# SutirthaChakraborty/RTFS-Net

Measured on AMD Instinct MI355X. Metric: mixtures/sec forward (2 s@16 kHz, 2-spk) RTFS-Net-4, higher is better.
Workload: dtype f32 (f16x3 split-precision MFMA products, f32 accumulate; every tensor in HBM is f32)

## Files before the change

rtfs-net_amd/csrc/api.hip:

```cpp
#include "api_common.h"
#include <atomic>
#include <vector>

namespace {

struct Cursor {
    const float* p;
    size_t off = 0;
    explicit Cursor(const float* base) : p(base) {}
    const float* take(size_t n) {
        const float* r = p ? p + off : nullptr;
        off += (n + 63) / 64 * 64;
        return r;
    }
};

struct Fork {
    hipStream_t st = nullptr;
    RtfsSide side{};
    bool open = false;
    int begin(hipStream_t owner, int slot) {
        st = owner;
        CHECK(rtfs_side_stream(owner, slot, &side));
        if (hipEventRecord(side.fork, st) != hipSuccess || hipStreamWaitEvent(side.stream, side.fork, 0) != hipSuccess) return RTFS_ERR_LAUNCH;
// ... 148 lines not shown
    explicit DecPack(Cursor& c) {
        wt = c.take(CA * 32);
        w16 = c.take(CA * 32);
        w16p = c.take(8192);
    }
};

inline bool gemm_f32() {
    static const bool v = [] {
        const char* e = getenv("RTFS_GEMM_F32");
        return e && e[0] == '1';
    }();
    return v;
}

DpArgs dp_args(const DpPack& p, const float* x, float* out, int R, int Ls, size_t bstride, size_t rstride, size_t cstride) {
    DpArgs a;
    a.x = x;
    a.out = out;
    a.R = R;
    a.Ls = Ls;
    a.bstride = bstride;
    a.rstride = rstride;
    a.cstride = cstride;
    a.ln_gamma = p.ln_g;
    a.ln_beta = p.ln_b;
    a.W0 = p.W0;
    a.Wl = p.Wl;
    a.wc = p.wc;
    a.bias = p.bias;
    a.Wt = p.Wt;
    a.bt = p.bt;
    a.whh = p.whh;
    return a;
}

Dp16Args dp16_args(const DpPack& p, const float* x, float* out, int nseq, int R, int Ls, size_t bstride, size_t rstride, size_t cstride) {
    Dp16Args a;
    a.x = x;
    a.out = out;
    a.nseq = nseq;
    a.R = R;
    a.Ls = Ls;
    a.bstride = bstride;
    a.rstride = rstride;
    a.cstride = cstride;
    a.ln_gamma = p.ln_g;
    a.ln_beta = p.ln_b;
    a.w16_l0 = reinterpret_cast<const half8*>(p.w16_l0);
    a.w16_l = reinterpret_cast<const half8*>(p.w16_l);
    a.w16_ct = reinterpret_cast<const half8*>(p.w16_ct);
    a.wf_l0 = reinterpret_cast<const half8*>(p.wf_l0);
    a.wf_l = reinterpret_cast<const half8*>(p.wf_l);
    a.wf_ct = reinterpret_cast<const half8*>(p.wf_ct);
    a.wc16 = p.wc16;
    a.bias16 = p.bias16;
    a.bt = p.bt;
    return a;
}

int dualpath(const DpPack& p, const float* x, float* out, int B, int T, int F, int dim, float* tA, float* tB, hipStream_t st) {
    const size_t plane = (size_t)T * F;
    if (dim == 4) {
        RTFS_RETURN_IF(F < 8 || F > 250, RTFS_ERR_SHAPE);
        if (!gemm_f32() && !p.whh) return launch_dualpath16(dp16_args(p, x, out, B * T, T, F, CH * plane, F, plane), st);
        return launch_dualpath(dp_args(p, x, out, T, F, CH * plane, F, plane), B * T, st);
    }
    RTFS_RETURN_IF(T < 8 || T > (p.whh ? 250 : 512), RTFS_ERR_SHAPE);
    CHECK(launch_transpose(x, tA, B * CH, T, F, st));
    if (T > 256 && !p.whh) {
        const int nb = (int)std::min<size_t>((size_t)B, (((size_t)1 << 32) - 1) / (CH * plane * sizeof(float)));
        for (int b0 = 0; b0 < B; b0 += nb) {
            const int n = std::min(nb, B - b0);
            CHECK(launch_dualpath16(dp16_args(p, tA + (size_t)b0 * CH * plane, tB + (size_t)b0 * CH * plane, n * F, F, T, CH * plane, T, plane), st));
        }
    } else if ((!gemm_f32() || T > 250) && !p.whh) {
        CHECK(launch_dualpath16(dp16_args(p, tA, tB, B * F, F, T, CH * plane, T, plane), st));
    } else {
        CHECK(launch_dualpath(dp_args(p, tA, tB, F, T, CH * plane, T, plane), B * F, st));
    }
    return launch_transpose(tB, out, B * CH, F, T, st);
}

int attention(const AttnPack& p, const float* x, float* out, int B, int T, float* q, float* k, float* v, float* o, hipStream_t st, bool cl = false) {
    RowCanArgs a;
    a.x = x;
    a.cl = cl;
    a.wt = p.qkv_wt;
    a.bias = p.qkv_b;
    a.slope = p.qkv_slope;
    a.gamma = p.qkv_gamma;
    a.beta = p.qkv_beta;
    a.ngroups = 12;
    for (int g = 0; g <= 12; ++g) a.group_start[g] = g <= 8 ? 4 * g : 32 + 16 * (g - 8);
    for (int g = 0; g < 12; ++g)
        for (int o_ = a.group_start[g]; o_ < a.group_start[g + 1]; ++o_) a.group_of[o_] = (unsigned char)g;
    a.T = T;
    a.q = q;
    a.k = k;
    a.v = v;
    CHECK(launch_row_can_qkv(a, B, st));
    AttnArgs c;
    c.q = q;
    c.k = k;
    c.v = v;
    c.out = o;
    c.T = T;
    c.scale = 1.0f / 16.0f;
    CHECK(launch_attn_core(c, B, st));
    RowCanArgs r;
    r.x = o;
    r.wt = p.proj_wt;
    r.bias = p.proj_b;
    r.slope = p.proj_slope;
    r.gamma = p.proj_gamma;
    r.beta = p.proj_beta;
    r.ngroups = 1;
    r.group_start[0] = 0;
    r.group_start[1] = 64;
    r.T = T;
    r.res = x;
    r.cl = cl;
    r.out = out;
    return launch_row_can_proj(r, B, st);
}

struct BlockWs {
    float *residual, *x_enc, *c0, *xf0, *expanded;
    float *c1, *p0, *g, *gF, *tA, *tB, *gT, *gA, *q, *k, *v, *o;
    float *E0, *G0, *E1, *G1, *L1, *xf1, *E2, *G2;
    double* stats;
    int Bfull = 0;
    int cs = 0;
    static constexpr int NSTAT = 11;
    enum { S_C0, S_C1, S_E0, S_G0, S_E1, S_G1, S_L1, S_E2, S_G2, S_L0, S_L2 };
    BlockWs(Arena& a, int B, int T, int F, int cs_ = 0) {
        const size_t Pg = (size_t)(T / 2) * (F / 2);
        cs = cs_ ? cs_ : T * F;
        const size_t P = (size_t)cs;
        Bfull = B;
        residual = a.take<float>(B * CA * P);
        x_enc = a.take<float>(B * CH * P);
        c0 = a.take<float>(B * CH * P);
        xf0 = a.take<float>(B * CH * P);
        expanded = a.take<float>(B * CH * P);
        float** gs[] = {&c1, &p0, &g, &gF, &tA, &tB, &gT, &gA, &v, &o, &E0, &G0, &E1, &G1, &L1, &xf1, &E2, &G2};
        for (float** s : gs) *s = a.take<float>(B * CH * Pg);
        q = a.take<float>(B * CH * Pg / 4);
        k = a.take<float>(B * CH * Pg / 4);
        stats = a.take<double>((size_t)NSTAT * B * 2);
    }
    double* st(int slot, int ) const { return stats ? stats + (size_t)slot * Bfull * 2 : nullptr; }
};

int block_head(const BlockPack& p, const float* x, const float* x_res, int B, int T, int F, BlockWs& w, hipStream_t st, const CafArgs* caf, unsigned* ctr = nullptr) {
    const int P = T * F;
    {
        PwArgs a;
        a.x = x;
        a.x2 = x_res;
        a.res_out = w.residual;
        a.wt = p.proj_wt;
        a.w16 = p.proj_w16;
        a.bias = p.proj_b;
        a.out = w.x_enc;
        a.gw = p.gw;
        a.gb = p.gb;
        a.slope = p.gslope;
        a.P = P;
        a.cs = w.cs;
        a.tile_ctr = ctr;
        if (caf && !gemm_f32()) {
            a.caf_r = caf->r_out; a.caf_att = caf->att_out;
            a.caf_w_key = caf->w_key; a.caf_bn_key = caf->bn_key; a.caf_w_val = caf->w_val; a.caf_bn_val = caf->bn_val;
            a.caf_T = caf->T; a.caf_F = caf->F; a.caf_Tv = caf->Tv;
        }
        if (gemm_f32()) return launch_pw_gateway_proj(a, B, st);
        const int rc = launch_pws_head4(a, B, st);
        if (rc == RTFS_ERR_ARG) CHECK(launch_pws_gateway_proj(a, B, st));
        else CHECK(rc);
    }
    return RTFS_OK;
}

int block_body(const BlockPack& p, int B, int T, int F, const BlockWs& w, hipStream_t st, bool zero_stats = true) {
    const int Tp = T / 2, Fp = F / 2;
    const int P = T * F, Pg = Tp * Fp;
    const double icF = 1.0 / ((double)CH * P), icG = 1.0 / ((double)CH * Pg);
    typedef BlockWs W;
    constexpr int TH_A = 24, TH_B = 24, TH_C = 12, TH_G = 64, TH_S = 64;
    if (zero_stats && hipMemsetAsync(w.stats, 0, sizeof(double) * W::NSTAT * w.Bfull * 2, st) != hipSuccess) return RTFS_ERR_LAUNCH;
    {
        DwArgs a;
        a.x = w.x_enc;
        a.w[0] = p.ds0_w;
        a.bias[0] = p.ds0_b;
        a.out[0] = w.c0;
        a.stats_out[0] = w.st(W::S_C0, B);
        a.C = CH; a.H = T; a.W = F; a.TH = TH_A; a.cs = w.cs;
        CHECK(launch_dw_s1(a, 1, false, 0, B, st));
    }
    DwArgs s14;
    s14.x = w.c0;
    s14.in_stats = w.st(W::S_C0, B); s14.in_inv_count = icF; s14.in_gamma = p.ds0_g; s14.in_beta = p.ds0_be;
    s14.C = CH; s14.H = T; s14.W = F; s14.TH = 64; s14.Hg = Tp; s14.Wg = Fp; s14.cs = w.cs;
    s14.w[0] = p.fus0.loc_w;
    s14.stats_out[0] = w.st(W::S_L0, B);
    s14.rev = 1;
    DwArgs s3;
    s3.x = w.c0;
    s3.in_stats = w.st(W::S_C0, B); s3.in_inv_count = icF; s3.in_gamma = p.ds0_g; s3.in_beta = p.ds0_be;
    s3.w[0] = p.ds1_w;
    s3.bias[0] = p.ds1_b;
    s3.out[0] = w.c1;
    s3.out[1] = w.p0;
    s3.stats_out[0] = w.st(W::S_C1, B);
    s3.C = CH; s3.H = T; s3.W = F; s3.Hg = Tp; s3.Wg = Fp; s3.TH = TH_C; s3.cs = w.cs;
    s3.rev = 1;
    {
        const int rc = launch_dw_s2_stats(s3, s14, B, st);
        if (rc != RTFS_OK) return rc == RTFS_ERR_ARG ? RTFS_ERR_SHAPE : rc;
    }
    CHECK(launch_g_form(w.p0, w.c1, w.st(W::S_C1, B), icG, p.ds1_g, p.ds1_be, w.g, B, CH, Pg, st));
    const size_t per = (size_t)CH * Pg;
    const int nb = (int)std::min<size_t>((size_t)B, (((size_t)1 << 32) - 1) / (per * sizeof(float)));
    const bool cl = !p.dpF.whh && !p.dpT.whh && !gemm_f32() && !dualpath_gen2() && Fp >= 8 && Fp <= 64 && Tp >= 8 && Tp <= 512 &&
                    nb >= 1 && (nb >= B || Tp > 256);
    if (cl) {
        for (int b0 = 0; b0 < B; b0 += nb) {
            const int n = std::min(nb, B - b0);
// ... 264 lines not shown
        case RTFS_PACK_ATTENTION: return pack_size<AttnPack>();
        case RTFS_PACK_TFAR: return pack_size<TfarPack>();
        case RTFS_PACK_CAF: return pack_size<CafPack>();
        case RTFS_PACK_S3: return pack_size<S3Pack>();
        case RTFS_PACK_DECODER: return pack_size<DecPack>();
    }
    return 0;
}

size_t rtfs_stft_encoder_workspace_bytes(int B, int L) { return (size_t)B * 2 * rtfs_num_frames(L) * NF * sizeof(float) + 256; }

int rtfs_stft_encoder_f32(const float* wav, const float* pack, float* a0, double* stats, int B, int L, void* ws, size_t ws_bytes, void* stream) {
    RTFS_RETURN_IF(!wav || !pack || !a0 || B < 1 || L <= 128, RTFS_ERR_ARG);
    const int T = rtfs_num_frames(L);
    Arena ar(ws, ws_bytes);
    float* spec = ar.take<float>((size_t)B * 2 * T * NF);
    RTFS_RETURN_IF(!ws || !ar.ok(), RTFS_ERR_WORKSPACE);
    Cursor c(pack);
    EncPack p(c);
    if (stats && hipMemsetAsync(stats, 0, sizeof(double) * 2 * B, S(stream)) != hipSuccess) return RTFS_ERR_LAUNCH;
    CHECK(launch_stft(wav, spec, B, L, T, S(stream)));
    return launch_enc_conv(spec, p.w, a0, stats, B, CA, T, NF, (size_t)T * NF, (size_t)CA * T * NF, S(stream));
}

size_t rtfs_audio_bottleneck_workspace_bytes(int B) { return sizeof(double) * 2 * B + 256; }

int rtfs_audio_bottleneck_f32(const float* x, const double* stats, const float* pack, float* out, int B, int T, int F, void* ws, size_t ws_bytes, void* stream) {
    RTFS_RETURN_IF(!x || !pack || !out || B < 1 || T < 1 || F < 1, RTFS_ERR_ARG);
    Cursor c(pack);
    BnPack p(c);
    if (!stats) {
        Arena ar(ws, ws_bytes);
        double* s = ar.take<double>(2 * B);
        RTFS_RETURN_IF(!ws || !ar.ok(), RTFS_ERR_WORKSPACE);
        if (hipMemsetAsync(s, 0, sizeof(double) * 2 * B, S(stream)) != hipSuccess) return RTFS_ERR_LAUNCH;
        CHECK(launch_stats(x, s, B, (size_t)CA * T * F, S(stream)));
        stats = s;
    }
    return audio_bn(p, x, stats, out, B, T * F, S(stream));
}

size_t rtfs_block_workspace_bytes(int B, int T, int F) {
    Arena ar(nullptr, 0);
    BlockWs w(ar, B, T, F);
    return ar.off + 256;
}

int rtfs_block_f32(const float* x, const float* x_res, const float* pack, float* out, int B, int T, int F, void* ws, size_t ws_bytes, void* stream, int rnn_kind) {
    RTFS_RETURN_IF(!x || !pack || !out, RTFS_ERR_ARG);
    RTFS_RETURN_IF(!shape_ok_block(B, T, F, rnn_kind), RTFS_ERR_SHAPE);
    Arena ar(ws, ws_bytes);
    BlockWs w(ar, B, T, F);
    RTFS_RETURN_IF(!ws || !ar.ok(), RTFS_ERR_WORKSPACE);
    RTFS_RETURN_IF(rnn_kind != 0 && rnn_kind != 1, RTFS_ERR_ARG);
    Cursor c(pack);
    BlockPack p = BlockPack::make(c, rnn_kind);
    return block_forward(p, x, x_res, out, B, T, F, w, S(stream));
}

size_t rtfs_dualpath_workspace_bytes(int B, int T, int F) { return 2 * ((size_t)B * CH * T * F * sizeof(float) + 256); }

int rtfs_dualpath_lstm_f32(const float* x, const float* pack, float* out, int B, int T, int F, int dim, void* ws, size_t ws_bytes, void* stream) {
    RTFS_RETURN_IF(!x || !pack || !out || B < 1 || (dim != 3 && dim != 4), RTFS_ERR_ARG);
    Arena ar(ws, ws_bytes);
    float* tA = ar.take<float>((size_t)B * CH * T * F);
    float* tB = ar.take<float>((size_t)B * CH * T * F);
    RTFS_RETURN_IF(dim == 3 && (!ws || !ar.ok()), RTFS_ERR_WORKSPACE);
    Cursor c(pack);
    DpPack p(c, 1);
    return dualpath(p, x, out, B, T, F, dim, tA, tB, S(stream));
}

int rtfs_dualpath_sru_f32(const float* x, const float* pack, float* out, int B, int T, int F, int dim, void* ws, size_t ws_bytes, void* stream) {
    RTFS_RETURN_IF(!x || !pack || !out || B < 1 || (dim != 3 && dim != 4), RTFS_ERR_ARG);
    Arena ar(ws, ws_bytes);
    float* tA = ar.take<float>((size_t)B * CH * T * F);
    float* tB = ar.take<float>((size_t)B * CH * T * F);
    RTFS_RETURN_IF(dim == 3 && (!ws || !ar.ok()), RTFS_ERR_WORKSPACE);
    Cursor c(pack);
    DpPack p(c);
    return dualpath(p, x, out, B, T, F, dim, tA, tB, S(stream));
}

size_t rtfs_tf_attention_workspace_bytes(int B, int T) { return (size_t)B * T * (4 * 256 + 4 * 256 + 4 * 1024 + 64 * FQ) * sizeof(float) + 4 * 256; }

int rtfs_tf_attention_f32(const float* x, const float* pack, float* out, int B, int T, void* ws, size_t ws_bytes, void* stream) {
    RTFS_RETURN_IF(!x || !pack || !out || B < 1, RTFS_ERR_ARG);
    RTFS_RETURN_IF(T < 1 || T > 512, RTFS_ERR_SHAPE);
    Arena ar(ws, ws_bytes);
    float* q = ar.take<float>((size_t)B * 4 * T * 256);
    float* k = ar.take<float>((size_t)B * 4 * T * 256);
    float* v = ar.take<float>((size_t)B * 4 * T * 1024);
    float* o = ar.take<float>((size_t)B * 64 * T * FQ);
    RTFS_RETURN_IF(!ws || !ar.ok(), RTFS_ERR_WORKSPACE);
    Cursor c(pack);
    AttnPack p(c);
    return attention(p, x, out, B, T, q, k, v, o, S(stream));
}

size_t rtfs_tfar_workspace_bytes(int B, int H, int W, int Hg, int Wg) {
    return 3 * ((size_t)B * CH * (size_t)(H * W > Hg * Wg ? Hg * Wg : H * W) * sizeof(float) + 256) + 3 * 2 * B * sizeof(double) + 256;
}

int rtfs_tfar_f32(const float* local, const float* global, const float* pack, float* out, int B, int H, int W, int Hg, int Wg, void* ws, size_t ws_bytes, void* stream) {
    RTFS_RETURN_IF(!local || !global || !pack || !out || B < 1, RTFS_ERR_ARG);
    const bool up = (size_t)H * W > (size_t)Hg * Wg;
    RTFS_RETURN_IF(!up && (H != Hg || W != Wg), RTFS_ERR_SHAPE);
    Arena ar(ws, ws_bytes);
    const size_t ng = (size_t)B * CH * Hg * Wg;
    float* E = ar.take<float>(ng);
    float* G = ar.take<float>(ng);
    float* Lc = ar.take<float>(ng);
    double* st = ar.take<double>(3 * 2 * B);
    RTFS_RETURN_IF(!ws || !ar.ok(), RTFS_ERR_WORKSPACE);
    Cursor c(pack);
    TfarPack p(c);
    hipStream_t s = S(stream);
    if (hipMemsetAsync(st, 0, sizeof(double) * 6 * B, s) != hipSuccess) return RTFS_ERR_LAUNCH;
    double *stE = st, *stG = st + 2 * B, *stL = st + 4 * B;
    const double icG = 1.0 / ((double)CH * Hg * Wg), icL = 1.0 / ((double)CH * H * W);
    {
        DwArgs a;
        a.x = global;
        a.w[0] = p.emb_w; a.w[1] = p.gate_w;
        a.out[0] = E; a.out[1] = G;
        a.stats_out[0] = stE; a.stats_out[1] = stG;
        a.C = CH; a.H = Hg; a.W = Wg; a.TH = 64;
        CHECK(launch_dw_s1(a, 2, false, 0, B, s));
    }
    if (up) {
        DwArgs a;
        a.x = local;
        a.w[0] = p.loc_w;
        a.C = CH; a.H = H; a.W = W; a.TH = 64; a.Hg = Hg; a.Wg = Wg;
        a.stats_out[0] = stL;
        CHECK(launch_dw_s1(a, 1, false, 1, B, s));
        a.stats_out[0] = nullptr;
        a.loc_stats = stL; a.loc_inv_count = icL; a.loc_gamma = p.loc_g; a.loc_beta = p.loc_b;
        a.gate = G; a.gate_stats = stG; a.gate_gamma = p.gate_g; a.gate_beta = p.gate_b;
        a.emb = E; a.emb_stats = stE; a.emb_gamma = p.emb_g; a.emb_beta = p.emb_b;
        a.g_inv_count = icG;
        a.out[0] = out;
        return launch_dw_s1(a, 1, false, 2, B, s);
    }
    {
        DwArgs a;
        a.x = local;
        a.w[0] = p.loc_w;
        a.out[0] = Lc;
        a.stats_out[0] = stL;
        a.C = CH; a.H = H; a.W = W; a.TH = 64;
        CHECK(launch_dw_s1(a, 1, false, 0, B, s));
    }
    GCombineArgs a;
    a.l = Lc; a.gate = G; a.emb = E;
    a.l_stats = stL; a.gate_stats = stG; a.emb_stats = stE;
    a.l_gamma = p.loc_g; a.l_beta = p.loc_b; a.gate_gamma = p.gate_g; a.gate_beta = p.gate_b; a.emb_gamma = p.emb_g; a.emb_beta = p.emb_b;
    a.inv_count = icG;
    a.out = out;
    a.C = CH; a.HW = H * W;
    return launch_g_combine(a, B, s);
}

size_t rtfs_caf_workspace_bytes(int B, int Tv) { return 2 * ((size_t)B * CA * Tv * sizeof(float) + 256); }

int rtfs_caf_f32(const float* audio, const float* video, const float* pack, float* out, int B, int T, int F, int Tv, void* ws, size_t ws_bytes, void* stream) {
    RTFS_RETURN_IF(!audio || !video || !pack || !out || B < 1 || T < 1 || F < 1 || Tv < 1, RTFS_ERR_ARG);
    Arena ar(ws, ws_bytes);
    float* r = ar.take<float>((size_t)B * CA * Tv);
    float* att = ar.take<float>((size_t)B * CA * Tv);
    RTFS_RETURN_IF(!ws || !ar.ok(), RTFS_ERR_WORKSPACE);
    Cursor c(pack);
    CafPack p(c);
    CafArgs a = caf_args(p, audio, video, out, r, att, T, F, Tv);
    CHECK(launch_caf_video(a, B, S(stream)));
// ... 410 lines not shown
```

rtfs-net_amd/csrc/k_attn.hip:

```cpp
#include "common.h"
#include "kernels.h"
#include "pipe_helpers.h"

#define AF 64

#define RCAN_ROWS 8
#define RCAN_LD 72
template <int NOUT, bool CL = false>
__global__ __launch_bounds__(256, 2) void row_can_kernel(RowCanArgs a) {
    constexpr int MT = NOUT / 32, MTW = (MT + 1) / 2;
    constexpr int NR = NOUT / 4;
    constexpr float WSC = 256.f, WINV = 1.f / 256.f;
    __shared__ float Ys[NOUT][RCAN_LD];
    __shared__ float bias_s[NOUT], slope_s[NOUT];
    __shared__ float red[8];
    constexpr bool XCL = CL && NOUT == 96, RCL = CL && NOUT == 64;
    __shared__ __attribute__((aligned(16))) float Rs[RCL ? AF : 1][RCL ? 68 : 4];
    const int T = a.T, b = blockIdx.y;
    const int tid = threadIdx.x, lane = tid & 63, r = lane & 31, h = lane >> 5;
    const int wave = __builtin_amdgcn_readfirstlane(tid >> 6);
    const int nt = wave & 1, mp = wave >> 1;
    for (int o = tid; o < NOUT; o += 256) {
        bias_s[o] = a.bias[o] * WSC;
        slope_s[o] = a.slope[NOUT == 96 ? a.group_of[o] : 0];
    }
    half8 wh[MTW][4], wl[MTW][4];
#pragma unroll
    for (int m = 0; m < MTW; ++m) {
        const int mt = min(mp + 2 * m, MT - 1);
#pragma unroll
        for (int ks = 0; ks < 4; ++ks)
#pragma unroll
            for (int j = 0; j < 8; ++j) {
                const float w = a.wt[(ks * 16 + 8 * h + j) * NOUT + mt * 32 + r] * WSC;
                const _Float16 hi = (_Float16)w;
                wh[m][ks][j] = hi;
                wl[m][ks][j] = (_Float16)(w - (float)hi);
            }
    }
    auto ln_row = [&](int i) -> int {
        if (NOUT == 64) return wave * 16 + i;
        return i < 4 ? 4 * wave + i : i < 8 ? 16 + 4 * wave + (i - 4) : 32 + 16 * wave + (i - 8);
    };
    __shared__ float gam_s[NOUT][AF], bet_s[NOUT][AF];
    for (int i = tid; i < NOUT * AF; i += 256) {
        gam_s[0][i] = a.gamma[i];
        bet_s[0][i] = a.beta[i];
    }
    const int t0 = blockIdx.x * a.rpw;
    const int nrows = min(a.rpw, T - t0);
    const float* __restrict__ X = XCL ? a.x + ((size_t)b * T * AF + nt * 32 + r) * 64 + 8 * h : a.x + (size_t)b * 64 * T * AF + nt * 32 + r;
    const float* __restrict__ RES = NOUT == 64 ? (RCL ? a.res + (size_t)b * T * AF * 64 + 4 * tid : a.res + ((size_t)b * 64 + wave * 16) * T * AF + lane)
                                               : nullptr;
    float v[4][8];
    float rs[NOUT == 64 ? 16 : 1];
    auto load_x = [&](int t) {
        if constexpr (XCL) {
#pragma unroll
            for (int ks = 0; ks < 4; ++ks) {
                *reinterpret_cast<f32x4*>(&v[ks][0]) = *reinterpret_cast<const f32x4*>(X + (size_t)t * AF * 64 + ks * 16);
                *reinterpret_cast<f32x4*>(&v[ks][4]) = *reinterpret_cast<const f32x4*>(X + (size_t)t * AF * 64 + ks * 16 + 4);
            }
        } else {
#pragma unroll
            for (int ks = 0; ks < 4; ++ks)
#pragma unroll
                for (int j = 0; j < 8; ++j) v[ks][j] = X[((size_t)(ks * 16 + 8 * h + j) * T + t) * AF];
        }
    };
    load_x(t0);
    __syncthreads();
    for (int rr = 0; rr < nrows; ++rr) {
        const int t = t0 + rr;
        half8 bh[4], bl[4];
#pragma unroll
        for (int ks = 0; ks < 4; ++ks) {
            unsigned hi[4], lo[4];
#pragma unroll
            for (int jp = 0; jp < 4; ++jp) split2(v[ks][2 * jp], v[ks][2 * jp + 1], hi[jp], lo[jp]);
            bh[ks] = __builtin_bit_cast(half8, *reinterpret_cast<f32x4*>(hi));
            bl[ks] = __builtin_bit_cast(half8, *reinterpret_cast<f32x4*>(lo));
        }
        if constexpr (RCL) {
#pragma unroll
            for (int k = 0; k < 4; ++k) *reinterpret_cast<f32x4*>(&rs[4 * k]) = *reinterpret_cast<const f32x4*>(RES + (size_t)t * AF * 64 + 1024 * k);
        } else if (NOUT == 64) {
#pragma unroll
            for (int i = 0; i < 16; ++i) rs[i] = RES[((size_t)i * T + t) * AF];
        }
        load_x(min(t + 1, T - 1));
#pragma unroll
        for (int m = 0; m < MTW; ++m) {
            const int mt = mp + 2 * m;
            if (mt < MT) {
                f32x16 acc;
#pragma unroll
                for (int q = 0; q < 16; ++q) acc[q] = bias_s[mt * 32 + (q & 3) + 8 * (q >> 2) + 4 * h];
#pragma unroll
                for (int ks = 0; ks < 4; ++ks) {
                    acc = __builtin_amdgcn_mfma_f32_32x32x16_f16(wh[m][ks], bh[ks], acc, 0, 0, 0);
                    acc = __builtin_amdgcn_mfma_f32_32x32x16_f16(wh[m][ks], bl[ks], acc, 0, 0, 0);
                    acc = __builtin_amdgcn_mfma_f32_32x32x16_f16(wl[m][ks], bh[ks], acc, 0, 0, 0);
                }
#pragma unroll
                for (int q = 0; q < 16; ++q) {
                    const int o = mt * 32 + (q & 3) + 8 * (q >> 2) + 4 * h;
                    Ys[o][nt * 32 + r] = preluf_(acc[q] * WINV, slope_s[o]);
                }
            }
        }
        if constexpr (RCL) {
#pragma unroll
            for (int k = 0; k < 4; ++k) *reinterpret_cast<f32x4*>(&Rs[tid / 16 + 16 * k][4 * (tid % 16)]) = *reinterpret_cast<const f32x4*>(&rs[4 * k]);
        }
        __syncthreads();
        float y[NR];
#pragma unroll
        for (int i = 0; i < NR; ++i) y[i] = Ys[ln_row(i)][lane];
        if (NOUT == 96) {
#pragma unroll
            for (int g = 0; g < 3; ++g) {
                const int i0 = g == 0 ? 0 : g == 1 ? 4 : 8, gs = g == 2 ? 16 : 4;
                float s = 0.f;
#pragma unroll
                for (int i = 0; i < gs; ++i) s += y[i0 + i];
                const float mean = wave_sum(s) / (float)(gs * AF);
                float vv = 0.f;
#pragma unroll
                for (int i = 0; i < gs; ++i) {
                    y[i0 + i] -= mean;
                    vv = fmaf(y[i0 + i], y[i0 + i], vv);
                }
                const float rstd = 1.0f / sqrtf(wave_sum(vv) / (float)(gs * AF) + RTFS_EPS);
                float* __restrict__ dst = (g == 0 ? a.q : g == 1 ? a.k : a.v) + (((size_t)b * 4 + wave) * T + t) * (gs * AF) + lane;
#pragma unroll
                for (int i = 0; i < gs; ++i) dst[i * AF] = fmaf(y[i0 + i] * rstd, gam_s[ln_row(i0 + i)][lane], bet_s[ln_row(i0 + i)][lane]);
            }
        } else {
            float s = 0.f;
#pragma unroll
            for (int i = 0; i < 16; ++i) s += y[i];
            s = wave_sum(s);
            if (lane == 0) red[wave] = s;
            __syncthreads();
            const float mean = (red[0] + red[1] + red[2] + red[3]) / (float)(64 * AF);
            float vv = 0.f;
#pragma unroll
            for (int i = 0; i < 16; ++i) {
                y[i] -= mean;
                vv = fmaf(y[i], y[i], vv);
            }
            vv = wave_sum(vv);
            if (lane == 0) red[4 + wave] = vv;
            __syncthreads();
            const float rstd = 1.0f / sqrtf((red[4] + red[5] + red[6] + red[7]) / (float)(64 * AF) + RTFS_EPS);
            float* __restrict__ O = a.out + ((size_t)b * 64 + wave * 16) * T * AF + lane;
            if constexpr (RCL) {
#pragma unroll
                for (int k = 0; k < 4; ++k) *reinterpret_cast<f32x4*>(&rs[4 * k]) = *reinterpret_cast<const f32x4*>(&Rs[lane][wave * 16 + 4 * k]);
            }
#pragma unroll
            for (int i = 0; i < 16; ++i) O[((size_t)i * T + t) * AF] = fmaf(y[i] * rstd, gam_s[ln_row(i)][lane], bet_s[ln_row(i)][lane]) + rs[i];
        }
        __syncthreads();
    }
}

#define ATT_PSC 4096.f
__device__ __forceinline__ void split8(const float (&v)[8], float sc, half8& hi, half8& lo) {
    unsigned h[4], l[4];
#pragma unroll
    for (int jp = 0; jp < 4; ++jp) split2(v[2 * jp] * sc, v[2 * jp + 1] * sc, h[jp], l[jp]);
    hi = __builtin_bit_cast(half8, *reinterpret_cast<f32x4*>(h));
    lo = __builtin_bit_cast(half8, *reinterpret_cast<f32x4*>(l));
}
__global__ __launch_bounds__(256) void attn_core_kernel(AttnArgs a) {
    extern __shared__ __attribute__((aligned(16))) float S[];
    const int T = a.T;
    const int NKT = (T + 31) >> 5;
    const int NK = NKT * 32;
    const int ldp = NK + 4;
    const int tid = threadIdx.x, lane = tid & 63, r = lane & 31, h = lane >> 5;
    const int wave = __builtin_amdgcn_readfirstlane(tid >> 6);
    const int nqt = (T + 31) >> 5;
    const int slot = blockIdx.x >> 3;
    const int pair = (slot / nqt) * 8 + (blockIdx.x & 7);
    if (pair >= a.npairs) return;
    const int q0 = (slot % nqt) * 32, hd = pair & 3, b = pair >> 2;
    const float* __restrict__ Q = a.q + ((size_t)b * 4 + hd) * T * 256;
    const float* __restrict__ K = a.k + ((size_t)b * 4 + hd) * T * 256;
    const float* __restrict__ V = a.v + ((size_t)b * 4 + hd) * T * 1024;

    for (int kg = 0; kg < NKT; kg += 8) {
        f32x16 acc[2];
#pragma unroll
        for (int j = 0; j < 2; ++j)
#pragma unroll
            for (int q = 0; q < 16; ++q) acc[j][q] = 0.f;
        const float* __restrict__ qp = Q + (size_t)min(q0 + r, T - 1) * 256 + 8 * h;
        const float* __restrict__ kp0 = K + (size_t)min((kg + wave) * 32 + r, T - 1) * 256 + 8 * h;
        const float* __restrict__ kp1 = K + (size_t)min((kg + wave + 4) * 32 + r, T - 1) * 256 + 8 * h;
        const bool two = kg + wave + 4 < NKT;
#pragma unroll 4
        for (int ks = 0; ks < 16; ++ks) {
            float qv[8], k0[8], k1[8];
            *reinterpret_cast<f32x4*>(qv) = *reinterpret_cast<const f32x4*>(qp + ks * 16);
            *reinterpret_cast<f32x4*>(qv + 4) = *reinterpret_cast<const f32x4*>(qp + ks * 16 + 4);
            *reinterpret_cast<f32x4*>(k0) = *reinterpret_cast<const f32x4*>(kp0 + ks * 16);
            *reinterpret_cast<f32x4*>(k0 + 4) = *reinterpret_cast<const f32x4*>(kp0 + ks * 16 + 4);
            *reinterpret_cast<f32x4*>(k1) = *reinterpret_cast<const f32x4*>(kp1 + ks * 16);
            *reinterpret_cast<f32x4*>(k1 + 4) = *reinterpret_cast<const f32x4*>(kp1 + ks * 16 + 4);
            half8 ah, al, bh, bl;
            split8(qv, 1.f, ah, al);
            split8(k0, 1.f, bh, bl);
            acc[0] = __builtin_amdgcn_mfma_f32_32x32x16_f16(ah, bh, acc[0], 0, 0, 0);
            acc[0] = __builtin_amdgcn_mfma_f32_32x32x16_f16(ah, bl, acc[0], 0, 0, 0);
            acc[0] = __builtin_amdgcn_mfma_f32_32x32x16_f16(al, bh, acc[0], 0, 0, 0);
            if (two) {
                split8(k1, 1.f, bh, bl);
                acc[1] = __builtin_amdgcn_mfma_f32_32x32x16_f16(ah, bh, acc[1], 0, 0, 0);
                acc[1] = __builtin_amdgcn_mfma_f32_32x32x16_f16(ah, bl, acc[1], 0, 0, 0);
                acc[1] = __builtin_amdgcn_mfma_f32_32x32x16_f16(al, bh, acc[1], 0, 0, 0);
            }
        }
#pragma unroll
        for (int j = 0; j < 2; ++j) {
            const int kt = kg + wave + 4 * j;
            if (kt < NKT) {
#pragma unroll
                for (int q = 0; q < 16; ++q) S[((q & 3) + 8 * (q >> 2) + 4 * h) * ldp + kt * 32 + r] = acc[j][q] * a.scale;
            }
        }
    }
    __syncthreads();
    for (int rr = 0; rr < 8; ++rr) {
        float* row = S + (wave * 8 + rr) * ldp;
        float m = -3.0e38f;
        for (int j = lane; j < T; j += 64) m = fmaxf(m, row[j]);
        m = wave_max(m);
        float s = 0.f;
        for (int j = lane; j < NK; j += 64) {
            const float e = j < T ? expf(row[j] - m) : 0.f;
            row[j] = e;
            s += e;
        }
        const float inv = 1.0f / wave_sum(s);
        for (int j = lane; j < NK; j += 64) row[j] *= inv;
    }
    __syncthreads();
    for (int grp = 0; grp < 2; ++grp) {
        f32x16 o[4];
#pragma unroll
        for (int n = 0; n < 4; ++n)
#pragma unroll
            for (int q = 0; q < 16; ++q) o[n][q] = 0.f;
        const int col0 = (wave * 8 + grp * 4) * 32 + 4 * r;
        const float* __restrict__ vp = V + col0;
        f32x4 vv[2][8];
        auto load_v = [&](int ks, f32x4 (&dst)[8]) {
#pragma unroll
            for (int j = 0; j < 8; ++j) dst[j] = *reinterpret_cast<const f32x4*>(vp + (size_t)min(ks * 16 + 8 * h + j, T - 1) * 1024);
        };
        auto step = [&](int ks, const f32x4 (&src)[8]) {
            float pv[8];
            *reinterpret_cast<f32x4*>(pv) = *reinterpret_cast<const f32x4*>(S + r * ldp + ks * 16 + 8 * h);
            *reinterpret_cast<f32x4*>(pv + 4) = *reinterpret_cast<const f32x4*>(S + r * ldp + ks * 16 + 8 * h + 4);
            half8 ph, pl;
            split8(pv, ATT_PSC, ph, pl);
#pragma unroll
            for (int n = 0; n < 4; ++n) {
                float t8[8];
#pragma unroll
                for (int j = 0; j < 8; ++j) t8[j] = src[j][n];
                half8 vh, vl;
                split8(t8, 1.f, vh, vl);
                o[n] = __builtin_amdgcn_mfma_f32_32x32x16_f16(ph, vh, o[n], 0, 0, 0);
                o[n] = __builtin_amdgcn_mfma_f32_32x32x16_f16(ph, vl, o[n], 0, 0, 0);
                o[n] = __builtin_amdgcn_mfma_f32_32x32x16_f16(pl, vh, o[n], 0, 0, 0);
            }
        };
        const int nks = NK / 16;
        load_v(0, vv[0]);
        for (int ks = 0; ks < nks; ks += 2) {
            load_v(ks + 1, vv[1]);
            step(ks, vv[0]);
            load_v(min(ks + 2, nks - 1), vv[0]);
            step(ks + 1, vv[1]);
        }
        {
            const int c = col0 >> 6, f = col0 & 63;
#pragma unroll
            for (int q = 0; q < 16; ++q) {
                const int qq = q0 + (q & 3) + 8 * (q >> 2) + 4 * h;
                if (qq < T)
                    *reinterpret_cast<f32x4*>(a.out + (((size_t)b * 64 + hd * 16 + c) * T + qq) * AF + f) =
                        f32x4{o[0][q], o[1][q], o[2][q], o[3][q]} * (1.f / ATT_PSC);
            }
        }
    }
}

size_t attn_core_lds_bytes(int T) {
    const int NK = ((T + 31) >> 5) * 32;
    return (size_t)32 * (NK + 4) * sizeof(float);
}

static int rcan_rows(int T, int B) {
    if ((long)T * B >= 3500) return RCAN_ROWS;
    const int r = (int)((long)T * B / 512);
    return r < 1 ? 1 : (r > RCAN_ROWS ? RCAN_ROWS : r);
}
int launch_row_can_qkv(const RowCanArgs& a_, int B, hipStream_t st) {
    RowCanArgs a = a_;
    a.rpw = rcan_rows(a.T, B);
    if (a.ngroups != 12 || a.group_start[8] != 32 || a.group_start[12] != 96) return RTFS_ERR_SHAPE;
    if (a.cl)
        hipLaunchKernelGGL((row_can_kernel<96, true>), dim3(cdiv(a.T, a.rpw), B), dim3(256), 0, st, a);
    else
        hipLaunchKernelGGL((row_can_kernel<96, false>), dim3(cdiv(a.T, a.rpw), B), dim3(256), 0, st, a);
    return rtfs_launch_status();
}
int launch_row_can_proj(const RowCanArgs& a_, int B, hipStream_t st) {
    RowCanArgs a = a_;
    a.rpw = rcan_rows(a.T, B);
    if (a.ngroups != 1) return RTFS_ERR_SHAPE;
    if (a.cl)
        hipLaunchKernelGGL((row_can_kernel<64, true>), dim3(cdiv(a.T, a.rpw), B), dim3(256), 0, st, a);
    else
        hipLaunchKernelGGL((row_can_kernel<64, false>), dim3(cdiv(a.T, a.rpw), B), dim3(256), 0, st, a);
    return rtfs_launch_status();
}
int launch_attn_core(const AttnArgs& a, int B, hipStream_t st) {
    if (a.T < 1 || a.T > 512) return RTFS_ERR_SHAPE;
    const size_t lds = attn_core_lds_bytes(a.T);
    if (rtfs_set_max_lds((const void*)attn_core_kernel, lds) != RTFS_OK) return RTFS_ERR_LAUNCH;
    AttnArgs a2 = a;
    a2.npairs = B * 4;
    hipLaunchKernelGGL(attn_core_kernel, dim3(cdiv(a2.npairs, 8) * 8 * cdiv(a.T, 32)), dim3(256), lds, st, a2);
    return rtfs_launch_status();
}
```

Measured before the change: 3308.

## Store attention Q/K/V pre-split as fp16 hi/lo pairs and restructure attention core

The QKV projection kernel now writes Q and K as interleaved fp16 hi/lo halves and V as row-paired fp16 hi/lo words, so the attention core no longer re-splits f32 values on every MFMA step. The attention core loads half8 operands directly, software-pipelines QK^T over K chunks, prefetches V three stages ahead, and stores softmax probabilities in LDS as fp16 hi/lo. The output projection now reads a transposed attention output layout. The aim is to cut the VALU split work and memory traffic in attention, at the cost of more complex layouts, higher register pressure with two blocks per CU, and odd-T handling in the V packing.

```diff
diff --git a/rtfs-net_amd/csrc/api.hip b/rtfs-net_amd/csrc/api.hip
--- a/rtfs-net_amd/csrc/api.hip
+++ b/rtfs-net_amd/csrc/api.hip
@@ -254,6 +254,7 @@
     return launch_transpose(tB, out, B * CH, F, T, st);
 }
 
+static size_t attn_v_rows(int T) { return ((size_t)T + 1) & ~(size_t)1; }
 int attention(const AttnPack& p, const float* x, float* out, int B, int T, float* q, float* k, float* v, float* o, hipStream_t st, bool cl = false) {
     RowCanArgs a;
     a.x = x;
@@ -316,8 +317,9 @@
         c0 = a.take<float>(B * CH * P);
         xf0 = a.take<float>(B * CH * P);
         expanded = a.take<float>(B * CH * P);
-        float** gs[] = {&c1, &p0, &g, &gF, &tA, &tB, &gT, &gA, &v, &o, &E0, &G0, &E1, &G1, &L1, &xf1, &E2, &G2};
+        float** gs[] = {&c1, &p0, &g, &gF, &tA, &tB, &gT, &gA, &o, &E0, &G0, &E1, &G1, &L1, &xf1, &E2, &G2};
         for (float** s : gs) *s = a.take<float>(B * CH * Pg);
+        v = a.take<float>(B * CH * attn_v_rows(T / 2) * (F / 2));
         q = a.take<float>(B * CH * Pg / 4);
         k = a.take<float>(B * CH * Pg / 4);
         stats = a.take<double>((size_t)NSTAT * B * 2);
@@ -748,7 +750,9 @@
     return dualpath(p, x, out, B, T, F, dim, tA, tB, S(stream));
 }
 
-size_t rtfs_tf_attention_workspace_bytes(int B, int T) { return (size_t)B * T * (4 * 256 + 4 * 256 + 4 * 1024 + 64 * FQ) * sizeof(float) + 4 * 256; }
+size_t rtfs_tf_attention_workspace_bytes(int B, int T) {
+    return (size_t)B * (T * (4 * 256 + 4 * 256 + 64 * FQ) + attn_v_rows(T) * 4 * 1024) * sizeof(float) + 4 * 256;
+}
 
 int rtfs_tf_attention_f32(const float* x, const float* pack, float* out, int B, int T, void* ws, size_t ws_bytes, void* stream) {
     RTFS_RETURN_IF(!x || !pack || !out || B < 1, RTFS_ERR_ARG);
@@ -756,7 +760,7 @@
     Arena ar(ws, ws_bytes);
     float* q = ar.take<float>((size_t)B * 4 * T * 256);
     float* k = ar.take<float>((size_t)B * 4 * T * 256);
-    float* v = ar.take<float>((size_t)B * 4 * T * 1024);
+    float* v = ar.take<float>((size_t)B * 4 * attn_v_rows(T) * 1024);
     float* o = ar.take<float>((size_t)B * 64 * T * FQ);
     RTFS_RETURN_IF(!ws || !ar.ok(), RTFS_ERR_WORKSPACE);
     Cursor c(pack);
diff --git a/rtfs-net_amd/csrc/k_attn.hip b/rtfs-net_amd/csrc/k_attn.hip
--- a/rtfs-net_amd/csrc/k_attn.hip
+++ b/rtfs-net_amd/csrc/k_attn.hip
@@ -11,10 +11,11 @@
     constexpr int MT = NOUT / 32, MTW = (MT + 1) / 2;
     constexpr int NR = NOUT / 4;
     constexpr float WSC = 256.f, WINV = 1.f / 256.f;
-    __shared__ float Ys[NOUT][RCAN_LD];
+    __shared__ __attribute__((aligned(16))) float Ys[NOUT][RCAN_LD];
     __shared__ float bias_s[NOUT], slope_s[NOUT];
     __shared__ float red[8];
     constexpr bool XCL = CL && NOUT == 96, RCL = CL && NOUT == 64;
+    constexpr bool XO = NOUT == 64;
     __shared__ __attribute__((aligned(16))) float Rs[RCL ? AF : 1][RCL ? 68 : 4];
     const int T = a.T, b = blockIdx.y;
     const int tid = threadIdx.x, lane = tid & 63, r = lane & 31, h = lane >> 5;
@@ -49,17 +50,26 @@
     }
     const int t0 = blockIdx.x * a.rpw;
     const int nrows = min(a.rpw, T - t0);
-    const float* __restrict__ X = XCL ? a.x + ((size_t)b * T * AF + nt * 32 + r) * 64 + 8 * h : a.x + (size_t)b * 64 * T * AF + nt * 32 + r;
+    const float* __restrict__ X = XCL  ? a.x + ((size_t)b * T * AF + nt * 32 + r) * 64 + 8 * h
+                                  : XO ? a.x + ((size_t)b * T * 16 + 2 * h) * 256 + (nt * 32 + r) * 4
+                                       : a.x + (size_t)b * 64 * T * AF + nt * 32 + r;
     const float* __restrict__ RES = NOUT == 64 ? (RCL ? a.res + (size_t)b * T * AF * 64 + 4 * tid : a.res + ((size_t)b * 64 + wave * 16) * T * AF + lane)
                                                : nullptr;
     float v[4][8];
     float rs[NOUT == 64 ? 16 : 1];
+    unsigned vst[NOUT == 96 ? 16 : 1];
     auto load_x = [&](int t) {
         if constexpr (XCL) {
 #pragma unroll
             for (int ks = 0; ks < 4; ++ks) {
                 *reinterpret_cast<f32x4*>(&v[ks][0]) = *reinterpret_cast<const f32x4*>(X + (size_t)t * AF * 64 + ks * 16);
                 *reinterpret_cast<f32x4*>(&v[ks][4]) = *reinterpret_cast<const f32x4*>(X + (size_t)t * AF * 64 + ks * 16 + 4);
+            }
+        } else if constexpr (XO) {
+#pragma unroll
+            for (int ks = 0; ks < 4; ++ks) {
+                *reinterpret_cast<f32x4*>(&v[ks][0]) = *reinterpret_cast<const f32x4*>(X + (size_t)t * 4096 + ks * 1024);
+                *reinterpret_cast<f32x4*>(&v[ks][4]) = *reinterpret_cast<const f32x4*>(X + (size_t)t * 4096 + ks * 1024 + 256);
             }
         } else {
 #pragma unroll
@@ -132,9 +142,55 @@
                     vv = fmaf(y[i0 + i], y[i0 + i], vv);
                 }
                 const float rstd = 1.0f / sqrtf(wave_sum(vv) / (float)(gs * AF) + RTFS_EPS);
-                float* __restrict__ dst = (g == 0 ? a.q : g == 1 ? a.k : a.v) + (((size_t)b * 4 + wave) * T + t) * (gs * AF) + lane;
-#pragma unroll
-                for (int i = 0; i < gs; ++i) dst[i * AF] = fmaf(y[i0 + i] * rstd, gam_s[ln_row(i0 + i)][lane], bet_s[ln_row(i0 + i)][lane]);
+                if (g < 2) {
+                    unsigned* __restrict__ dst = reinterpret_cast<unsigned*>(g == 0 ? a.q : a.k) + (((size_t)b * 4 + wave) * T + t) * 256 + (lane & 1) * 128 + (lane >> 1);
+                    const unsigned sel = (lane & 1) ? 0x03020706u : 0x05040100u;
+#pragma unroll
+                    for (int i = 0; i < 4; i += 2) {
+                        unsigned hi, lo;
+                        split2(fmaf(y[i0 + i] * rstd, gam_s[ln_row(i0 + i)][lane], bet_s[ln_row(i0 + i)][lane]),
+                               fmaf(y[i0 + i + 1] * rstd, gam_s[ln_row(i0 + i + 1)][lane], bet_s[ln_row(i0 + i + 1)][lane]), hi, lo);
+                        const unsigned w0 = (hi & 0xffffu) | (lo << 16), w1 = (hi >> 16) | (lo & 0xffff0000u);
+                        dst[i * 32] = __builtin_amdgcn_perm(__builtin_amdgcn_mov_dpp(w0, 0xB1, 0xF, 0xF, true), w0, sel);
+                        dst[(i + 1) * 32] = __builtin_amdgcn_perm(__builtin_amdgcn_mov_dpp(w1, 0xB1, 0xF, 0xF, true), w1, sel);
+                    }
+                } else {
+                    unsigned w[16];
+#pragma unroll
+                    for (int i = 0; i < 16; i += 2) {
+                        unsigned hi, lo;
+                        split2(fmaf(y[8 + i] * rstd, gam_s[ln_row(8 + i)][lane], bet_s[ln_row(8 + i)][lane]),
+                               fmaf(y[9 + i] * rstd, gam_s[ln_row(9 + i)][lane], bet_s[ln_row(9 + i)][lane]), hi, lo);
+                        w[i] = (hi & 0xffffu) | (lo << 16);
+                        w[i + 1] = (hi >> 16) | (lo & 0xffff0000u);
+                    }
+                    unsigned* __restrict__ dst = reinterpret_cast<unsigned*>(a.v) + ((((size_t)b * 4 + wave) * ((T + 1) >> 1)) + (t >> 1)) * 2048 + lane * 4;
+                    const bool odd = t & 1;
+                    if (!odd && rr + 1 < nrows) {
+#pragma unroll
+                        for (int i = 0; i < 16; ++i) vst[i] = w[i];
+                    } else if (odd ? rr > 0 : t == T - 1) {
+#pragma unroll
+                        for (int k = 0; k < 4; ++k) {
+                            u32x4 ph, pl;
+#pragma unroll
+                            for (int c = 0; c < 4; ++c) {
+                                const unsigned e = odd ? vst[4 * k + c] : w[4 * k + c], o = odd ? w[4 * k + c] : 0u;
+                                ph[c] = (e & 0xffffu) | (o << 16);
+                                pl[c] = (e >> 16) | (o & 0xffff0000u);
+                            }
+                            *reinterpret_cast<u32x4*>(dst + k * 256) = ph;
+                            *reinterpret_cast<u32x4*>(dst + 1024 + k * 256) = pl;
+                        }
+                    } else {
+                        unsigned short* __restrict__ d16 = reinterpret_cast<unsigned short*>(dst) + odd;
+#pragma unroll
+                        for (int i = 0; i < 16; ++i) {
+                            d16[((i >> 2) * 256 + (i & 3)) * 2] = (unsigned short)w[i];
+                            d16[(1024 + (i >> 2) * 256 + (i & 3)) * 2] = (unsigned short)(w[i] >> 16);
+                        }
+                    }
+                }
             }
         } else {
             float s = 0.f;
@@ -167,14 +223,7 @@
 }
 
 #define ATT_PSC 4096.f
-__device__ __forceinline__ void split8(const float (&v)[8], float sc, half8& hi, half8& lo) {
-    unsigned h[4], l[4];
-#pragma unroll
-    for (int jp = 0; jp < 4; ++jp) split2(v[2 * jp] * sc, v[2 * jp + 1] * sc, h[jp], l[jp]);
-    hi = __builtin_bit_cast(half8, *reinterpret_cast<f32x4*>(h));
-    lo = __builtin_bit_cast(half8, *reinterpret_cast<f32x4*>(l));
-}
-__global__ __launch_bounds__(256) void attn_core_kernel(AttnArgs a) {
+__global__ __launch_bounds__(256, 2) void attn_core_kernel(AttnArgs a) {
     extern __shared__ __attribute__((aligned(16))) float S[];
     const int T = a.T;
     const int NKT = (T + 31) >> 5;
@@ -187,116 +236,137 @@
     const int pair = (slot / nqt) * 8 + (blockIdx.x & 7);
     if (pair >= a.npairs) return;
     const int q0 = (slot % nqt) * 32, hd = pair & 3, b = pair >> 2;
-    const float* __restrict__ Q = a.q + ((size_t)b * 4 + hd) * T * 256;
-    const float* __restrict__ K = a.k + ((size_t)b * 4 + hd) * T * 256;
-    const float* __restrict__ V = a.v + ((size_t)b * 4 + hd) * T * 1024;
-
-    for (int kg = 0; kg < NKT; kg += 8) {
-        f32x16 acc[2];
-#pragma unroll
-        for (int j = 0; j < 2; ++j)
-#pragma unroll
-            for (int q = 0; q < 16; ++q) acc[j][q] = 0.f;
-        const float* __restrict__ qp = Q + (size_t)min(q0 + r, T - 1) * 256 + 8 * h;
-        const float* __restrict__ kp0 = K + (size_t)min((kg + wave) * 32 + r, T - 1) * 256 + 8 * h;
-        const float* __restrict__ kp1 = K + (size_t)min((kg + wave + 4) * 32 + r, T - 1) * 256 + 8 * h;
-        const bool two = kg + wave + 4 < NKT;
-#pragma unroll 4
-        for (int ks = 0; ks < 16; ++ks) {
-            float qv[8], k0[8], k1[8];
-            *reinterpret_cast<f32x4*>(qv) = *reinterpret_cast<const f32x4*>(qp + ks * 16);
-            *reinterpret_cast<f32x4*>(qv + 4) = *reinterpret_cast<const f32x4*>(qp + ks * 16 + 4);
-            *reinterpret_cast<f32x4*>(k0) = *reinterpret_cast<const f32x4*>(kp0 + ks * 16);
-            *reinterpret_cast<f32x4*>(k0 + 4) = *reinterpret_cast<const f32x4*>(kp0 + ks * 16 + 4);
-            *reinterpret_cast<f32x4*>(k1) = *reinterpret_cast<const f32x4*>(kp1 + ks * 16);
-            *reinterpret_cast<f32x4*>(k1 + 4) = *reinterpret_cast<const f32x4*>(kp1 + ks * 16 + 4);
-            half8 ah, al, bh, bl;
-            split8(qv, 1.f, ah, al);
-            split8(k0, 1.f, bh, bl);
-            acc[0] = __builtin_amdgcn_mfma_f32_32x32x16_f16(ah, bh, acc[0], 0, 0, 0);
-            acc[0] = __builtin_amdgcn_mfma_f32_32x32x16_f16(ah, bl, acc[0], 0, 0, 0);
-            acc[0] = __builtin_amdgcn_mfma_f32_32x32x16_f16(al, bh, acc[0], 0, 0, 0);
-            if (two) {
-                split8(k1, 1.f, bh, bl);
-                acc[1] = __builtin_amdgcn_mfma_f32_32x32x16_f16(ah, bh, acc[1], 0, 0, 0);
-                acc[1] = __builtin_amdgcn_mfma_f32_32x32x16_f16(ah, bl, acc[1], 0, 0, 0);
-                acc[1] = __builtin_amdgcn_mfma_f32_32x32x16_f16(al, bh, acc[1], 0, 0, 0);
-            }
-        }
-#pragma unroll
-        for (int j = 0; j < 2; ++j) {
-            const int kt = kg + wave + 4 * j;
-            if (kt < NKT) {
-#pragma unroll
-                for (int q = 0; q < 16; ++q) S[((q & 3) + 8 * (q >> 2) + 4 * h) * ldp + kt * 32 + r] = acc[j][q] * a.scale;
-            }
-        }
-    }
+    const _Float16* __restrict__ Q = reinterpret_cast<const _Float16*>(a.q) + ((size_t)b * 4 + hd) * T * 512;
+    const _Float16* __restrict__ K = reinterpret_cast<const _Float16*>(a.k) + ((size_t)b * 4 + hd) * T * 512;
+    const int T2 = (T + 1) >> 1;
+    const unsigned* __restrict__ V = reinterpret_cast<const unsigned*>(a.v) + ((size_t)b * 4 + hd) * T2 * 2048;
+
+    {
+        const int ng = wave < NKT ? ((NKT - wave + 3) >> 2) * 4 : 0;
+        const _Float16* __restrict__ qp = Q + (size_t)min(q0 + r, T - 1) * 512 + 8 * h;
+        half8 sb[2][16];
+        f32x16 acc;
+        auto load_s = [&](int g, half8 (&dst)[16]) {
+            if (g < ng) {
+                const int k0 = (g & 3) * 64;
+                const _Float16* __restrict__ kp = K + (size_t)min((wave + (g & ~3)) * 32 + r, T - 1) * 512 + 8 * h + k0;
+#pragma unroll
+                for (int kk = 0; kk < 4; ++kk) {
+                    dst[4 * kk] = *reinterpret_cast<const half8*>(qp + k0 + kk * 16);
+                    dst[4 * kk + 1] = *reinterpret_cast<const half8*>(qp + k0 + kk * 16 + 256);
+                    dst[4 * kk + 2] = *reinterpret_cast<const half8*>(kp + kk * 16);
+                    dst[4 * kk + 3] = *reinterpret_cast<const half8*>(kp + kk * 16 + 256);
+                }
+            }
+        };
+        auto step_s = [&](int g, const half8 (&src)[16]) {
+            if ((g & 3) == 0) {
+#pragma unroll
+                for (int q = 0; q < 16; ++q) acc[q] = 0.f;
+            }
+#pragma unroll
+            for (int kk = 0; kk < 4; ++kk) {
+                acc = __builtin_amdgcn_mfma_f32_32x32x16_f16(src[4 * kk], src[4 * kk + 2], acc, 0, 0, 0);
+                acc = __builtin_amdgcn_mfma_f32_32x32x16_f16(src[4 * kk], src[4 * kk + 3], acc, 0, 0, 0);
+                acc = __builtin_amdgcn_mfma_f32_32x32x16_f16(src[4 * kk + 1], src[4 * kk + 2], acc, 0, 0, 0);
+            }
+            if ((g & 3) == 3) {
+                const int kt = wave + (g & ~3);
+#pragma unroll
+                for (int q = 0; q < 16; ++q) S[((q & 3) + 8 * (q >> 2) + 4 * h) * ldp + kt * 32 + r] = acc[q] * a.scale;
+            }
+        };
+        load_s(0, sb[0]);
+        for (int g = 0; g < ng; g += 2) {
+            load_s(g + 1, sb[1]);
+            step_s(g, sb[0]);
+            load_s(g + 2, sb[0]);
+            step_s(g + 1, sb[1]);
+        }
+    }
+    const int nks = NK / 16, nst = 2 * nks;
+    u32x4 vb[4][8];
+    auto load_v = [&](int s, u32x4 (&dst)[8]) {
+        if (s < nst) {
+            const int grp = s >= nks, ks = s - grp * nks, g = wave * 2 + grp;
+            const unsigned* __restrict__ vp = V + ((g >> 1) * 64 + (g & 1) * 32 + r) * 4;
+#pragma unroll
+            for (int jj = 0; jj < 4; ++jj) {
+                const size_t pr = (size_t)min(ks * 8 + 4 * h + jj, T2 - 1) * 2048;
+                dst[2 * jj] = *reinterpret_cast<const u32x4*>(vp + pr);
+                dst[2 * jj + 1] = *reinterpret_cast<const u32x4*>(vp + pr + 1024);
+            }
+        }
+    };
+    load_v(0, vb[0]);
+    load_v(1, vb[1]);
+    load_v(2, vb[2]);
     __syncthreads();
     for (int rr = 0; rr < 8; ++rr) {
         float* row = S + (wave * 8 + rr) * ldp;
         float m = -3.0e38f;
         for (int j = lane; j < T; j += 64) m = fmaxf(m, row[j]);
         m = wave_max(m);
+        float e[8];
         float s = 0.f;
-        for (int j = lane; j < NK; j += 64) {
-            const float e = j < T ? expf(row[j] - m) : 0.f;
-            row[j] = e;
-            s += e;
+#pragma unroll
+        for (int p = 0; p < 8; ++p) {
+            const int j = lane + 64 * p;
+            e[p] = j < T ? expf(row[j] - m) : 0.f;
+            s += e[p];
         }
         const float inv = 1.0f / wave_sum(s);
-        for (int j = lane; j < NK; j += 64) row[j] *= inv;
+        unsigned short* rh = reinterpret_cast<unsigned short*>(row);
+#pragma unroll
+        for (int p = 0; p < 8; ++p) {
+            const int j = lane + 64 * p;
+            if (j < NK) {
+                unsigned hi, lo;
+                split2(e[p] * inv * ATT_PSC, 0.f, hi, lo);
+                rh[j] = (unsigned short)hi;
+                rh[NK + j] = (unsigned short)lo;
+            }
+        }
     }
     __syncthreads();
-    for (int grp = 0; grp < 2; ++grp) {
-        f32x16 o[4];
-#pragma unroll
-        for (int n = 0; n < 4; ++n)
-#pragma unroll
-            for (int q = 0; q < 16; ++q) o[n][q] = 0.f;
-        const int col0 = (wave * 8 + grp * 4) * 32 + 4 * r;
-        const float* __restrict__ vp = V + col0;
-        f32x4 vv[2][8];
-        auto load_v = [&](int ks, f32x4 (&dst)[8]) {
-#pragma unroll
-            for (int j = 0; j < 8; ++j) dst[j] = *reinterpret_cast<const f32x4*>(vp + (size_t)min(ks * 16 + 8 * h + j, T - 1) * 1024);
-        };
-        auto step = [&](int ks, const f32x4 (&src)[8]) {
-            float pv[8];
-            *reinterpret_cast<f32x4*>(pv) = *reinterpret_cast<const f32x4*>(S + r * ldp + ks * 16 + 8 * h);
-            *reinterpret_cast<f32x4*>(pv + 4) = *reinterpret_cast<const f32x4*>(S + r * ldp + ks * 16 + 8 * h + 4);
-            half8 ph, pl;
-            split8(pv, ATT_PSC, ph, pl);
-#pragma unroll
-            for (int n = 0; n < 4; ++n) {
-                float t8[8];
-#pragma unroll
-                for (int j = 0; j < 8; ++j) t8[j] = src[j][n];
-                half8 vh, vl;
-                split8(t8, 1.f, vh, vl);
-                o[n] = __builtin_amdgcn_mfma_f32_32x32x16_f16(ph, vh, o[n], 0, 0, 0);
-                o[n] = __builtin_amdgcn_mfma_f32_32x32x16_f16(ph, vl, o[n], 0, 0, 0);
-                o[n] = __builtin_amdgcn_mfma_f32_32x32x16_f16(pl, vh, o[n], 0, 0, 0);
-            }
-        };
-        const int nks = NK / 16;
-        load_v(0, vv[0]);
-        for (int ks = 0; ks < nks; ks += 2) {
-            load_v(ks + 1, vv[1]);
-            step(ks, vv[0]);
-            load_v(min(ks + 2, nks - 1), vv[0]);
-            step(ks + 1, vv[1]);
-        }
-        {
-            const int c = col0 >> 6, f = col0 & 63;
+    f32x16 o[4];
+    auto step = [&](int s, const u32x4 (&src)[8]) {
+        const int grp = s >= nks, ks = s - grp * nks;
+        if (ks == 0) {
+#pragma unroll
+            for (int n = 0; n < 4; ++n)
+#pragma unroll
+                for (int q = 0; q < 16; ++q) o[n][q] = 0.f;
+        }
+        const _Float16* pr = reinterpret_cast<const _Float16*>(S + r * ldp) + ks * 16 + 8 * h;
+        const half8 ph = *reinterpret_cast<const half8*>(pr), pl = *reinterpret_cast<const half8*>(pr + NK);
+#pragma unroll
+        for (int n = 0; n < 4; ++n) {
+            const half8 vh = __builtin_bit_cast(half8, u32x4{src[0][n], src[2][n], src[4][n], src[6][n]});
+            const half8 vl = __builtin_bit_cast(half8, u32x4{src[1][n], src[3][n], src[5][n], src[7][n]});
+            o[n] = __builtin_amdgcn_mfma_f32_32x32x16_f16(ph, vh, o[n], 0, 0, 0);
+            o[n] = __builtin_amdgcn_mfma_f32_32x32x16_f16(ph, vl, o[n], 0, 0, 0);
+            o[n] = __builtin_amdgcn_mfma_f32_32x32x16_f16(pl, vh, o[n], 0, 0, 0);
+        }
+        if (ks == nks - 1) {
+            const int g = wave * 2 + grp;
+            float* __restrict__ op = a.out + (((size_t)b * T * 16 + hd * 4 + (g >> 1)) * 64 + (g & 1) * 32 + r) * 4;
 #pragma unroll
             for (int q = 0; q < 16; ++q) {
                 const int qq = q0 + (q & 3) + 8 * (q >> 2) + 4 * h;
-                if (qq < T)
-                    *reinterpret_cast<f32x4*>(a.out + (((size_t)b * 64 + hd * 16 + c) * T + qq) * AF + f) =
-                        f32x4{o[0][q], o[1][q], o[2][q], o[3][q]} * (1.f / ATT_PSC);
-            }
-        }
+                if (qq < T) *reinterpret_cast<f32x4*>(op + (size_t)qq * 4096) = f32x4{o[0][q], o[1][q], o[2][q], o[3][q]} * (1.f / ATT_PSC);
+            }
+        }
+    };
+    for (int s = 0; s < nst; s += 4) {
+        load_v(s + 3, vb[3]);
+        step(s, vb[0]);
+        load_v(s + 4, vb[0]);
+        step(s + 1, vb[1]);
+        load_v(s + 5, vb[1]);
+        step(s + 2, vb[2]);
+        load_v(s + 6, vb[2]);
+        step(s + 3, vb[3]);
     }
 }
 
```

After: 3323 (median of 6 runs). No clear change (+0.4%).
